# Artessay/RAGraph

Measured on AMD Instinct MI355X. Metric: retrieved-queries/sec (RAGraph_node forward: GCN encode + cosine/top-k retrieval + 3-hop propagate + decode), higher is better.
Workload: dtype f32 (exact results; candidates pre-filtered on bf16 / int8 MFMA with proven bounds)

## Files before the change

ragraph_amd/csrc/filter_prepare.h:

```cpp

constexpr int FILTER_STATS_INTS = 32;
constexpr int FILTER_STATS_MAGIC = 0x52414753;
__device__ __forceinline__ void note_candidates(int* cstat, int64_t b, int n) {
  if (cstat && (b & 63) == 0) {
    atomicAdd(cstat, n);
    atomicAdd(cstat + 3, 1);
  }
}
struct FilterStatsInit {
  int nlev, i8[3], keys[3];
};

constexpr int FILTER_FIX_MAX_Q = 1024;
constexpr int FILTER_FIX_SLICES = 16;

template <int D, int R = 1>
__global__ void __launch_bounds__(256) filter_prep_kernel(const float* __restrict__ Q, int64_t B, float* __restrict__ Qn,
                                                          float* __restrict__ eq, int* __restrict__ count,
                                                          unsigned char* __restrict__ flag, int* __restrict__ overflow,
                                                          int* __restrict__ gmax, int ngroups,
                                                          uint16_t* __restrict__ Qb, int cstride,
                                                          float* __restrict__ eq8, float* __restrict__ qscale,
                                                          signed char* __restrict__ Qb8, int* __restrict__ fix_done,
                                                          int* __restrict__ stats, FilterStatsInit si,
                                                          float* __restrict__ theta_init, float prior) {
  const int lane = threadIdx.x & 63;
  constexpr int NCH = D / 4;
  const int64_t q_first = ((int64_t)blockIdx.x * 4 + (threadIdx.x >> 6)) * R;
  float4 vpre[R];
#pragma unroll
  for (int rr = 0; rr < R; ++rr) {
    vpre[rr] = make_float4(0.f, 0.f, 0.f, 0.f);
    if (lane < NCH && q_first + rr < B) vpre[rr] = reinterpret_cast<const float4*>(Q + (q_first + rr) * D)[lane];
  }
#pragma unroll
  for (int rr = 0; rr < R; ++rr) {
  const int64_t q = q_first + rr;
  if (q == 0 && lane == 0) *overflow = 0;
  if (q == 0 && lane < FILTER_STATS_INTS && stats) {
    int v = 0;
    if (lane == 0) v = FILTER_STATS_MAGIC;
    else if (lane == 1) v = si.nlev;
    else if (lane >= 8 && lane < 11) v = si.i8[lane - 8];
    else if (lane >= 11 && lane < 14) v = si.keys[lane - 11];
    else if (lane == 14) v = B > INT_MAX ? INT_MAX : (int)B;
    else if (lane == 16) v = theta_init ? 1 : 0;
    else if (lane == 18) v = INT_MAX;
    else if (lane == 19) v = INT_MIN;
    stats[lane] = v;
  }
  if (theta_init && q < B && lane == 0) theta_init[q] = prior;
  if (q < FILTER_FIX_MAX_Q && lane == 0) fix_done[q] = 0;
  if (q >= (Qb ? (B + 31) / 32 * 32 : B)) continue;
  float4 v = vpre[rr];
  float p = 0.f;
  p = fmaf(v.x, v.x, p);
  p = fmaf(v.y, v.y, p);
  p = fmaf(v.z, v.z, p);
  p = fmaf(v.w, v.w, p);
  p = wave_sum_fixed_tree(p);
  const float d = fmaxf(sqrtf(p), 1e-12f);
  v.x = v.x / d; v.y = v.y / d; v.z = v.z / d; v.w = v.w / d;
  if (lane < NCH && q < B) reinterpret_cast<float4*>(Qn + q * D)[lane] = v;
  if (Qb && lane < NCH) {
    const int e0 = 4 * lane, t = e0 >> 5, gg = (e0 >> 3) & 3;
    typedef __bf16 bf16x4 __attribute__((ext_vector_type(4)));
    bf16x4 o;
    o[0] = (__bf16)v.x; o[1] = (__bf16)v.y; o[2] = (__bf16)v.z; o[3] = (__bf16)v.w;
    char* base = reinterpret_cast<char*>(Qb) + ((q >> 4) * (D / 32) + t) * 1024 + (gg * 16 + (int)(q & 15)) * 16 + (e0 & 7) * 2;
    *reinterpret_cast<bf16x4*>(base) = o;
  }
  float e2 = 0.f;
  {
    const float x[4] = {v.x, v.y, v.z, v.w};
#pragma unroll
    for (int e = 0; e < 4; ++e) {
      const float dd = x[e] - (float)(__bf16)x[e];
      e2 = fmaf(dd, dd, e2);
    }
  }
  e2 = wave_sum_any_order(e2);
  float e8 = 0.f, sq = 0.f;
  unsigned am = max(max(__float_as_uint(fabsf(v.x)), __float_as_uint(fabsf(v.y))), max(__float_as_uint(fabsf(v.z)), __float_as_uint(fabsf(v.w))));
  am = wave_max_u32(am);
  if (eq8) {
    sq = __uint_as_float(am) / 127.f;
    unsigned w8 = 0u;
    if (sq > 0.f) {
      const float x[4] = {v.x, v.y, v.z, v.w};
#pragma unroll
      for (int e = 0; e < 4; ++e) {
        const int qi = quantize_i8(x[e], 1.f / sq);
        w8 |= ((unsigned)qi & 0xFFu) << (8 * e);
        const float dd = fmaf(sq, (float)qi, -x[e]);
        e8 = fmaf(dd, dd, e8);
      }
    }
    if (Qb8 && lane < NCH) {
      const int c = lane >> 2;
      char* base = reinterpret_cast<char*>(Qb8) + ((q >> 4) * (D / 64) + (c >> 2)) * 1024 + ((c & 3) * 16 + (int)(q & 15)) * 16 + (lane & 3) * 4;
      *reinterpret_cast<unsigned*>(base) = w8;
    }
    e8 = wave_sum_any_order(e8);
  }
  if (q >= B) continue;
  if (lane == 0) {
    eq[q] = sqrtf(e2) * 1.0000002f;
    flag[q] = am == 0u ? 2 : 0;
    if (am == 0u && stats) atomicAdd(stats + 15, 1);
    if (eq8) {
      eq8[q] = sqrtf(e8) * 1.000001f;
      qscale[q] = sq;
    }
  }
  if (lane < cstride) count[q * cstride + lane] = 0;
  if (gmax)
    for (int gi = lane; gi < ngroups; gi += 64) gmax[q * ngroups + gi] = f2ord(RG_NEG_INF);
  }
}

__global__ void __launch_bounds__(256) filter_theta_kernel(FilterThr t, int64_t B, int init, float* __restrict__ theta) {
  const int64_t q = (int64_t)blockIdx.x * 256 + threadIdx.x;
// ... 78 lines not shown
```

ragraph_amd/csrc/filter_ring.h:

```cpp

#ifdef RG_RING_STAMPS
__device__ unsigned long long g_ring_t[2][2][8];
__device__ unsigned long long g_ring_span[2][2];
__device__ unsigned long long g_ring_max[2][8];
#define RG_RSTAMP(i_)                                                                                     \
  if (threadIdx.x == 0 && first_seg) {                                                                    \
    const unsigned long long now_ = wall_clock64();                                                       \
    if (blockIdx.x == 0 || blockIdx.x == gridDim.x - 1) g_ring_t[BOUND][blockIdx.x != 0][i_] = now_;      \
    if ((i_) == 0) atomicMin(&g_ring_span[BOUND][0], now_);                                               \
    else atomicMax(&g_ring_max[BOUND][i_], now_ - rs_prev);                                               \
    rs_prev = now_;                                                                                       \
  }
static void ring_stamps_report(bool BOUND, bool I8) {
  (void)hipDeviceSynchronize();
  unsigned long long t[2][2][8];
  (void)hipMemcpyFromSymbol(t, HIP_SYMBOL(g_ring_t), sizeof(t));
  for (int b = 0; b < 2; ++b)
    fprintf(stderr, "[ring stamps, %s%s launch, %s workgroup, 10 ns ticks] operands %lld thresholds %lld ring primed %lld stages %lld "
            "flush %lld (entered %lld after workgroup 0)\n", BOUND ? "bound" : "filter", I8 ? " int8" : "", b ? "last" : "first",
            (long long)(t[BOUND][b][1] - t[BOUND][b][0]), (long long)(t[BOUND][b][2] - t[BOUND][b][1]),
            (long long)(t[BOUND][b][3] - t[BOUND][b][2]), (long long)(t[BOUND][b][4] - t[BOUND][b][3]),
            (long long)(t[BOUND][b][5] - t[BOUND][b][4]), (long long)(t[BOUND][b][0] - t[BOUND][0][0]));
  unsigned long long span[2][2], mx[2][8];
  (void)hipMemcpyFromSymbol(span, HIP_SYMBOL(g_ring_span), sizeof(span));
  (void)hipMemcpyFromSymbol(mx, HIP_SYMBOL(g_ring_max), sizeof(mx));
  fprintf(stderr, "[ring stamps, all workgroups] first entry to last exit %lld; longest first-segment phases: operands %lld thresholds %lld "
          "ring primed %lld stages %lld flush %lld\n", (long long)(span[BOUND][1] - span[BOUND][0]), (long long)mx[BOUND][1],
          (long long)mx[BOUND][2], (long long)mx[BOUND][3], (long long)mx[BOUND][4], (long long)mx[BOUND][5]);
  unsigned long long init_span[2][2] = {{~0ull, 0ull}, {~0ull, 0ull}}, zero[2][8] = {};
  (void)hipMemcpyToSymbol(HIP_SYMBOL(g_ring_span), init_span, sizeof(init_span));
  (void)hipMemcpyToSymbol(HIP_SYMBOL(g_ring_max), zero, sizeof(zero));
}
#else
#define RG_RSTAMP(i_)
static void ring_stamps_report(bool, bool) {}
#endif
#ifdef RG_TOPK_TIMING
__device__ unsigned long long g_filter_timing[8];
#define RG_FT(var_) const unsigned long long var_ = __builtin_amdgcn_s_memtime()
static void ring_timing_report(int prof_slot, int D) {
  (void)hipDeviceSynchronize();
  unsigned long long t[8];
  (void)hipMemcpyFromSymbol(t, HIP_SYMBOL(g_filter_timing), sizeof(t));
  const double n = (double)t[5];
  if (n > 0)
    fprintf(stderr, "[filter timing] slot %d D=%d wave-stages=%.0f ticks/stage: wait_full %.1f compute %.1f signal+vmcnt "
            "%.1f wait_free %.1f dma_issue %.1f total %.1f; flushes in the loop: %.0f, %.1f ticks each = %.1f per stage\n",
            prof_slot, D, n, t[0] / n, t[1] / n, t[2] / n, t[3] / n, t[4] / n, (t[0] + t[1] + t[2] + t[3] + t[4]) / n, (double)t[7],
            t[7] ? (double)t[6] / (double)t[7] : 0.0, t[6] / n);
  unsigned long long zero[8] = {0, 0, 0, 0, 0, 0, 0, 0};
  (void)hipMemcpyToSymbol(HIP_SYMBOL(g_filter_timing), zero, sizeof(zero));
}
#else
#define RG_FT(var_)
static void ring_timing_report(int, int) {}
#endif

#ifndef RG_RING_FOLD
#define RG_RING_FOLD 1
#endif
template <int D, int QW, bool BOUND = false, bool I8 = false, bool SCORED = false, bool PIPE = false>
__global__ void __launch_bounds__(512, 2) topk_filter_kernel(FilterParams p) {
  using C = FilterCfg<I8 ? D / 2 : D>;
  static_assert(!PIPE || (I8 && !BOUND && C::KSTEPS >= QW / 16 + 2), "PIPE: int8 filter levels, one step per query group + 2");
  static_assert(!(I8 && BOUND), "the bound pass runs on the bf16 copy");
  static_assert(I8 || !SCORED, "scored lists carry the int8 levels' integer sums");
  static_assert(QW == 32 || QW == 64 || QW == 96 || QW == 128, "two, four, six or eight query groups of 16 per wave");
  constexpr int QT = C::WAVES * QW;
  constexpr int NG = QW / 16;
  constexpr bool FOLD = RG_RING_FOLD && I8 && !PIPE && !BOUND && D == 64;
  if (filter_gate_closed(p.gate)) return;
  extern __shared__ float4 fsmem4[];
  char* smem = reinterpret_cast<char*>(fsmem4);
  unsigned* full = reinterpret_cast<unsigned*>(smem + C::SLOTS * C::STAGE_BYTES);
  unsigned* freec = full + C::SLOTS;
  const unsigned lds_base = (unsigned)(size_t)(lds_void_f*)smem;

  const int tid = threadIdx.x;
  const int lane = tid & 63;
  const int wave = __builtin_amdgcn_readfirstlane(tid >> 6);
  const int j = lane & 15, g = lane >> 4;

  unsigned voff[C::DMAS];
#pragma unroll
  for (int i = 0; i < C::DMAS; ++i) voff[i] = (unsigned)(i * 1024 + lane * 16);
  auto dma_stage = [&](int64_t stage_abs, int slot) {
    const uint64_t goff = (uint64_t)stage_abs * C::STAGE_BYTES + (uint64_t)(C::DMAS * wave * 1024);
    const char* gbase = reinterpret_cast<const char*>(p.Kb) +
                        (((uint64_t)(unsigned)__builtin_amdgcn_readfirstlane((int)(goff >> 32)) << 32) |
                         (uint64_t)(unsigned)__builtin_amdgcn_readfirstlane((int)(unsigned)goff));
#pragma unroll
    for (int i = 0; i < C::DMAS; ++i) {
      const unsigned dst = lds_base + (unsigned)(slot * C::STAGE_BYTES + (C::DMAS * wave + i) * 1024);
      unsigned keep;
      asm volatile(
          "s_mov_b32 %0, m0\n\ts_mov_b32 m0, %2\n\ts_nop 0\n\tglobal_load_lds_dwordx4 %1, %3\n\ts_mov_b32 m0, %0"
          : "=&s"(keep)
          : "v"(voff[i]), "s"(dst), "s"(gbase)
          : "memory");
    }
  };
  const unsigned apos = lds_base + (unsigned)lane * 16u;

  const int x = p.xcd_map ? (int)(blockIdx.x & 7) : 0;
  const int64_t nq = p.xcd_map ? ((p.qtiles - x + 7) >> 3) : p.qtiles;
  const int64_t nq0 = p.xcd_map ? ((p.qtiles + 7) >> 3) : p.qtiles;
  SegmentWalker walker(nq, p.nstages_total, p.wgs_per_group, p.lb_min, 0, p.depth[nq != nq0],
                       p.xcd_map ? (int)(blockIdx.x >> 3) : (int)blockIdx.x);
  Segment seg;
  [[maybe_unused]] bool first_seg = true;
#ifdef RG_RING_STAMPS
  unsigned long long rs_prev = 0;
#endif
  RG_RSTAMP(0);
  while (walker.next(seg)) {
    const int64_t qtile = p.xcd_map ? x + 8 * seg.tile : seg.tile;
    const int64_t q_lo = qtile * QT + wave * QW + j;
    const int64_t st0 = seg.st0;
    const int nstages = (int)(seg.st1 - seg.st0);

    bf16x8 bq[I8 ? 1 : NG][I8 ? 1 : C::KS32];
    i32x4 bqi[I8 ? NG : 1][I8 ? C::KS32 : 1];
    constexpr int TB = C::KS32 < 4 ? C::KS32 : 4;
    if constexpr (I8) {
      if (p.Qb) {
        const int64_t qg0 = (qtile * QT + wave * QW) >> 4;
        const int64_t ngroups16 = ((p.B + 31) / 32 * 32) >> 4;
#pragma unroll
        for (int gq = 0; gq < NG; ++gq) {
          const bool have = qg0 + gq < ngroups16;
          const i32x4* src = reinterpret_cast<const i32x4*>(p.Qb) + ((qg0 + gq) * C::KS32) * 64 + lane;
#pragma unroll
          for (int t = 0; t < C::KS32; ++t) {
            i32x4 z = {0, 0, 0, 0};
            bqi[gq][t] = have ? src[t * 64] : z;
          }
        }
      } else
#pragma unroll
      for (int gq = 0; gq < NG; ++gq) {
        const int64_t qq = q_lo + 16 * gq;
        const int64_t qr = qq < p.B ? qq : p.B - 1;
        const float sq = p.thr.qscale[qr];
        const float inv_sq = sq > 0.f ? 1.f / sq : 0.f;
        const float* r0 = p.Qn + qr * D + 16 * g;
#pragma unroll
        for (int t = 0; t < C::KS32; ++t) {
          float4 u[4];
#pragma unroll
          for (int c = 0; c < 4; ++c) u[c] = *reinterpret_cast<const float4*>(r0 + 64 * t + 4 * c);
#pragma unroll
          for (int c = 0; c < 4; ++c) {
            unsigned w = 0u;
            if (sq > 0.f)
              w = ((unsigned)quantize_i8(u[c].x, inv_sq) & 0xFFu) | (((unsigned)quantize_i8(u[c].y, inv_sq) & 0xFFu) << 8) |
                  (((unsigned)quantize_i8(u[c].z, inv_sq) & 0xFFu) << 16) | (((unsigned)quantize_i8(u[c].w, inv_sq) & 0xFFu) << 24);
            bqi[gq][t][c] = (int)w;
          }
          asm volatile("" : "+v"(bqi[gq][t]));
        }
        asm volatile("" ::: "memory");
      }
    } else if (p.Qb) {
      const int64_t qg0 = (qtile * QT + wave * QW) >> 4;
      const int64_t ngroups16 = ((p.B + 31) / 32 * 32) >> 4;
#pragma unroll
      for (int gq = 0; gq < NG; ++gq) {
        const bool have = qg0 + gq < ngroups16;
        const bf16x8* src = reinterpret_cast<const bf16x8*>(p.Qb) + ((qg0 + gq) * C::KS32) * 64 + lane;
#pragma unroll
        for (int t = 0; t < C::KS32; ++t) {
          bf16x8 z;
#pragma unroll
          for (int e = 0; e < 8; ++e) z[e] = (__bf16)0.f;
          bq[gq][t] = have ? src[t * 64] : z;
        }
      }
    } else
#pragma unroll
    for (int gq = 0; gq < NG; ++gq) {
      const int64_t qq = q_lo + 16 * gq;
      const float* r0 = p.Qn + (qq < p.B ? qq : p.B - 1) * D + 8 * g;
#pragma unroll
      for (int t0 = 0; t0 < C::KS32; t0 += TB) {
#pragma unroll
        for (int t = t0; t < t0 + TB; ++t) {
          const float4 u0 = *reinterpret_cast<const float4*>(r0 + 32 * t), u1 = *reinterpret_cast<const float4*>(r0 + 32 * t + 4);
          bq[gq][t][0] = (__bf16)u0.x; bq[gq][t][1] = (__bf16)u0.y; bq[gq][t][2] = (__bf16)u0.z; bq[gq][t][3] = (__bf16)u0.w;
          bq[gq][t][4] = (__bf16)u1.x; bq[gq][t][5] = (__bf16)u1.y; bq[gq][t][6] = (__bf16)u1.z; bq[gq][t][7] = (__bf16)u1.w;
        }
#pragma unroll
        for (int t = t0; t < t0 + TB; ++t) asm volatile("" : "+v"(bq[gq][t]));
        asm volatile("" ::: "memory");
      }
    }
    RG_RSTAMP(1);
    float thr[NG];
    int thr8[NG], thr8h[NG];
#pragma unroll
// ... 459 lines not shown
```

ragraph_amd/csrc/segment_plan.h:

```cpp
#pragma once
#include <stdint.h>

#if defined(__HIPCC__)
#define RG_HD __host__ __device__
#else
#define RG_HD
#endif

namespace ragraph {

struct Segment {
  int64_t tile;
  int64_t st0, st1;
  int slot;
  int last;
};

struct SegmentWalker {
  static constexpr int MIN_SHARE = 4;

  int64_t NS;
  int W, c, lb_min, warm, depth;
  int64_t rounds, round;
  int64_t t0, nT, c0, nC, lo, hi, bud;
// ... 97 lines not shown
        s.st1 = lo + take;
        s.slot = slot0;
        s.last = (lo + take == hi);
        c0 += nT;
        nC -= nT;
        lo += take;
        ++slot0;
        if (carry + take + warm > worst) worst = carry + take + warm;
        if (lo >= hi) nT = 0;
        if (mine) {
          phase = 3;
          return true;
        }
      }
    }
    if (phase == 2) {
      const int64_t len = hi - lo;
      if (aligned) {
        phase = 3;
        const int64_t ci = c - c0;
        if (ci < 0) return false;
        const int64_t jt = ci / m, piece = ci % m;
        const int64_t a = piece * per;
        if (jt >= nT || a >= len) return false;
        s.tile = t0 + jt;
        s.st0 = lo + a;
        s.st1 = a + per < len ? lo + a + per : hi;
        s.slot = slot0 + (int)piece;
        s.last = (s.st1 == hi);
        return true;
      }
      if (c < c0 || lin >= lin_end) {
        phase = 3;
        return false;
      }
      const int64_t jt = lin / len;
      const int64_t a = lin - jt * len;
      const int64_t b = (a + (lin_end - lin) < len) ? a + (lin_end - lin) : len;
      s.tile = t0 + jt;
      s.st0 = lo + a;
      s.st1 = lo + b;
      s.slot = slot0 + (int)((c - c0) - (jt * len) / Lb);
      s.last = (lo + b == hi);
      lin += b - a;
      return true;
    }
    return false;
  }

  struct Choice {
    int depth;
    int64_t slots;
    int64_t load;
  };

  static inline Choice choose_depth(int64_t nq, int64_t NS, int W, int lb_min, int warm) {
    Choice best = {0, 1, 0};
    int64_t min_load = -1;
    int64_t loads[80], slots[80];
    int nd = 0;
    for (int d = 0; d < 80; ++d) {
      SegmentWalker w(nq, NS, W, lb_min, warm, d, -1);
      Segment s;
      while (w.next(s)) {
      }
      loads[d] = w.worst;
      slots[d] = w.used;
      nd = d + 1;
      if (min_load < 0 || w.worst < min_load) min_load = w.worst;
      if (w.steps < d) break;
    }
    const int64_t whole = (nq / W) * (NS + warm) + min_load;
    for (int d = nd - 1; d >= 0; --d)
      if (loads[d] <= min_load + whole / 256) {
        best.depth = d;
        best.slots = slots[d];
        best.load = loads[d];
        break;
      }
    return best;
  }
};

}
```

ragraph_amd/csrc/topk_filter.hip:

```cpp
#include "filter_common.h"
#include "rescore_common.h"
#include <new>
#include "segment_plan.h"
#include <cmath>
#include <type_traits>

namespace ragraph {

typedef __attribute__((address_space(3))) void lds_void_f;
typedef int i32x4 __attribute__((ext_vector_type(4)));

template <int D_>
struct FilterCfg {
  static constexpr int D = D_;
  static constexpr int WAVES = 8, THREADS = 512;
  static constexpr int ROW_BYTES = D * 2;
  static constexpr int CR = D / 8;
  static constexpr int KSTEPS = D / 16;
  static constexpr int KS32 = D / 32;
  static constexpr int STAGE_BYTES = FILTER_STAGE_BYTES;
  static constexpr int STAGE_KEYS = STAGE_BYTES / ROW_BYTES;
  static constexpr int SUBS = STAGE_KEYS / 32;
  static constexpr int NSTEP = SUBS * KSTEPS;
  static constexpr int SLOTS = 4;
// ... 259 lines not shown
  f.part_s = B <= 64 ? reinterpret_cast<float*>(take((size_t)B * 8 * k * sizeof(float))) : nullptr;
  f.part_i = B <= 64 ? reinterpret_cast<int*>(take((size_t)B * 8 * k * sizeof(int))) : nullptr;
  f.eq8 = reinterpret_cast<float*>(take((size_t)B * sizeof(float)));
  f.qscale = reinterpret_cast<float*>(take((size_t)B * sizeof(float)));
  f.Qb8 = B <= FILTER_QB_MAX_B ? reinterpret_cast<signed char*>(take((size_t)((B + 31) / 32 * 32) * D)) : nullptr;
  if (out) *out = f;
  return off;
}

static int filter_shape_code(int64_t B, int64_t N, int D, int k) {
  if (!filter_dim_ok(D)) return RAGRAPH_EUNSUPPORTED;
  return B >= 1 && N >= 1 && k >= 1 && k <= 32 && k <= N ? RAGRAPH_OK : RAGRAPH_EINVAL;
}
#define RG_REQUIRE_FILTER_SHAPE(who, B, N, D, k)                                                                      \
  do {                                                                                                                \
    const int code__ = filter_shape_code(B, N, D, k);                                                                 \
    RG_REQUIRE(code__ != RAGRAPH_EUNSUPPORTED, RAGRAPH_EUNSUPPORTED, who ": D=%d not in {64,128,256}", D);           \
    RG_REQUIRE(code__ == RAGRAPH_OK, RAGRAPH_EINVAL, who ": bad B/N/k");                                              \
  } while (0)

static FilterShape filter_query_shape(int64_t B, int64_t N, int D, int k, int n_shards, bool exchange) {
  return {B, N, N, D, k, n_shards, exchange, __builtin_nanf(""), -1, false, filter_env(), filter_device_cus(), __builtin_nanf("")};
}
static void filter_query_follow_tight(FilterShape& in) {
  if (t_prior == t_prior && t_tight == t_tight && t_tight > t_prior) {
    in.prior = t_prior;
    in.tight = t_tight;
  }
}

static size_t filter_workspace_bytes(FilterShape in, const FilterSchedule& sc) {
  const FilterCall planned = filter_call_plan(in, sc);
  in.exact_level0 = true;
  const FilterCall exact0 = filter_call_plan(in, sc);
  return (planned.level0_bytes > exact0.level0_bytes ? planned.level0_bytes : exact0.level0_bytes) +
         filter_ws_carve(nullptr, in, planned, nullptr) + FILTER_STATS_BYTES;
}
static size_t filter_workspace_bytes(int64_t B, int64_t N, int D, int k, int n_shards) {
  if (B < 1 || N < 1 || k < 1 || n_shards < 1 || !filter_dim_ok(D)) return 0;
  const FilterShape in = filter_query_shape(B, N, D, k, n_shards, n_shards > 1);
  return filter_workspace_bytes(in, filter_schedule(in));
}

extern "C" size_t ragraph_topk_cosine_filtered_workspace_bytes(int64_t B, int64_t N, int D, int k) {
  return filter_workspace_bytes(B, N, D, k, 1);
}
extern "C" size_t ragraph_topk_cosine_filtered_sharded_workspace_bytes(int64_t B, int64_t plan_N, int D, int k, int n_shards) {
  if (!filter_dim_ok(D)) return 0;
  const size_t a = filter_workspace_bytes(B, plan_N, D, k, n_shards), b = filter_workspace_bytes(B, plan_N, D, k, 1);
  const size_t c = ragraph_topk_cosine_workspace_bytes(B, plan_N, D, k);
  const size_t ab = a > b ? a : b;
  return ab > c ? ab : c;
}

extern "C" int ragraph_topk_cosine_filtered_i8_levels(int64_t B, int64_t N, int D, int k) {
  if (filter_shape_code(B, N, D, k) != RAGRAPH_OK) return 0;
  FilterShape in = filter_query_shape(B, N, D, k, 1, false);
  in.i8_cap = t_max_i8_levels;
  filter_query_follow_tight(in);
  return filter_call_plan(in, filter_schedule(in)).i8_levels;
}

extern "C" int ragraph_topk_cosine_filtered_plan(int64_t B, int64_t N, int D, int k, int64_t plan[7]) {
  RG_REQUIRE(plan, RAGRAPH_EINVAL, "topk_cosine_filtered_plan: null pointer");
  RG_REQUIRE_FILTER_SHAPE("topk_cosine_filtered_plan", B, N, D, k);
  FilterShape in = filter_query_shape(B, N, D, k, 1, false);
  filter_query_follow_tight(in);
  const FilterCall c = filter_call_plan(in, filter_schedule(in));
  plan[0] = c.n0;
  plan[1] = c.level0 == FILTER_L0_BOUND ? 2 : (c.level0 == FILTER_L0_SLAB ? 1 : 0);
  plan[2] = c.nlev;
  for (int l = 0; l < FILTER_MAX_LEVELS; ++l) plan[3 + l] = l < c.nlev ? c.level[l].key1 : 0;
  plan[6] = c.bound_keys;
  return c.nlev;
}

extern "C" int ragraph_topk_cosine_filtered_sharded_speculates(int64_t B, int64_t plan_N, int D, int k, int n_shards) {
  if (filter_shape_code(B, plan_N, D, k) != RAGRAPH_OK || n_shards < 1) return 0;
  FilterShape in = filter_query_shape(B, plan_N, D, k, n_shards, true);
  in.prior = 0.f;
  return filter_call_plan(in, filter_schedule(in)).spec ? 1 : 0;
}

template <int D, int QW, bool BOUND, bool I8 = false, bool SCORED = false, bool PIPE = false>
static int launch_ring(FilterParams p, int64_t B, int CUS, int prof_slot, hipStream_t st) {
  using C = FilterCfg<I8 ? D / 2 : D>;
  p.qtiles = cdiv(B, (int64_t)C::WAVES * QW);
  p.xcd_map = p.qtiles >= 64 ? 1 : 0;
  p.wgs_per_group = CUS / (p.xcd_map ? 8 : 1);
  {
    const int64_t per_wg = p.qtiles * p.nstages_total / CUS;
    p.lb_min = per_wg >= 16 ? 8 : (per_wg >= 8 ? 4 : (per_wg >= 3 ? 2 : 1));
  }
  const int64_t nq0 = p.xcd_map ? (p.qtiles + 7) / 8 : p.qtiles;
  for (int v = 0; v < 2; ++v) {
    const int64_t nq = nq0 - v;
    p.depth[v] = 0;
    if (nq < 1 || (v == 1 && (!p.xcd_map || p.qtiles % 8 == 0))) continue;
    p.depth[v] = SegmentWalker::choose_depth(nq, p.nstages_total, p.wgs_per_group, p.lb_min, 0).depth;
    if (p.qtiles * p.nstages_total / CUS < 16) p.depth[v] = 0;
  }
  static DeviceOnce lds_once;
  if (hipError_t e = raise_dynamic_lds(lds_once, &topk_filter_kernel<D, QW, BOUND, I8, SCORED, PIPE>, (int)C::LDS_BYTES); e != hipSuccess) {
    set_error("topk_cosine_filtered: cannot raise dynamic LDS limit: %s", hipGetErrorString(e));
    return RAGRAPH_EDEVICE;
  }
  if (t_prof && prof_slot >= 0) (void)hipEventRecord(t_prof->ev[2 * prof_slot], st);
  hipLaunchKernelGGL((topk_filter_kernel<D, QW, BOUND, I8, SCORED, PIPE>), dim3((unsigned)CUS), dim3(C::THREADS), C::LDS_BYTES, st, p);
  if (t_prof && prof_slot >= 0) (void)hipEventRecord(t_prof->ev[2 * prof_slot + 1], st);
  RG_CHECK_LAUNCH("topk_cosine_filtered(filter)");
  ring_stamps_report(BOUND, I8);
  if (prof_slot >= 0) ring_timing_report(prof_slot, D);
  return RAGRAPH_OK;
}

struct PassVariant {
  bool direct;
  int qw;
  bool bound, i8, scored, pipe;
};
static PassVariant filter_pass_variant(int D, int64_t B, int64_t key0, int64_t key1, bool bound, bool int8, bool scored, int cus,
                                       const FilterEnv& env) {
  PassVariant v{};
  v.qw = 64;
  v.bound = bound;
  v.i8 = int8;
  v.scored = int8 && scored;
  if (B <= 256) {
    v.direct = true;
    return v;
  }
  const int64_t nstages = cdiv(key1 - key0, FILTER_STAGE_BYTES / ((int8 ? 1 : 2) * D));
  auto long_stream = [&](int64_t tile) { return cdiv(B, tile) * nstages >= 32 * (int64_t)cus; };
  if (!int8) {
    if (!bound && D == 64 && B >= 1024 && long_stream(1024)) v.qw = 128;
    return v;
  }
  const int64_t pad64 = cdiv(B, (int64_t)512) * 512 - B;
  auto fits = [&](int64_t tile) {
    return long_stream(tile) && (cdiv(B, tile) * tile - B - pad64) * 50 <= B;
  };
  const int qw = env.i8_qw ? env.i8_qw : (D == 64 && fits(1024) ? 128 : (fits(768) ? 96 : 64));
  const bool long128 = qw == 128 && long_stream(1024), long96 = qw == 96 && long_stream(768);
  if (D == 256 && ((env.pipe == 1 && !long128 && !long96) || env.pipe == 2)) v.pipe = true;
  else v.qw = long128 ? 128 : (long96 ? 96 : 64);
  return v;
}

template <int D>
static int launch_ring_variant(const PassVariant& v, const FilterParams& p, int64_t B, int cus, int prof_slot, hipStream_t st) {
  RG_REQUIRE(!v.direct && (v.qw == 64 || (v.i8 ? !v.pipe && (v.qw == 96 || v.qw == 128) : D == 64 && !v.bound && v.qw == 128)) &&
             (!v.pipe || (D == 256 && v.i8)), RAGRAPH_EINVAL, "topk_cosine_filtered: no ring kernel for D=%d qw=%d bound=%d int8=%d pipe=%d",
             D, v.qw, (int)v.bound, (int)v.i8, (int)v.pipe);
  if (v.bound) return launch_ring<D, 64, true>(p, B, cus, prof_slot, st);
  if (!v.i8) {
    if constexpr (D == 64)
      if (v.qw == 128) return launch_ring<D, 128, false>(p, B, cus, prof_slot, st);
    return launch_ring<D, 64, false>(p, B, cus, prof_slot, st);
  }
  if constexpr (D == 256)
    if (v.pipe)
      return v.scored ? launch_ring<D, 64, false, true, true, true>(p, B, cus, prof_slot, st)
                      : launch_ring<D, 64, false, true, false, true>(p, B, cus, prof_slot, st);
#define RG_RING_I8(QW_) \
  return v.scored ? launch_ring<D, QW_, false, true, true>(p, B, cus, prof_slot, st) : launch_ring<D, QW_, false, true>(p, B, cus, prof_slot, st)
  if (v.qw == 128) RG_RING_I8(128);
  if (v.qw == 96) RG_RING_I8(96);
  RG_RING_I8(64);
#undef RG_RING_I8
}

template <int D>
static int run_pass(const FilterWs& f, const uint16_t* Kb, const signed char* Kb8, int64_t B, int64_t key0, int64_t key1,
                    const FilterThr& thr, int cap, int bound_groups, bool int8, bool scored, const FilterEnv& env, int cus,
                    int prof_slot, hipStream_t st, FilterGate gate = FilterGate{nullptr, 0, 0}) {
  const PassVariant v = filter_pass_variant(D, B, key0, key1, bound_groups > 0, int8, scored, cus, env);
  const uint16_t* keys = v.i8 ? reinterpret_cast<const uint16_t*>(Kb8) : Kb;
  const uint16_t* Qimg = v.i8 ? reinterpret_cast<const uint16_t*>(f.Qb8) : f.Qb;
  if (v.direct) {
    DirectArgs a{};
    a.Qb = Qimg;
    a.Kb = keys;
    a.i8 = v.i8;
    a.scored = v.scored;
// ... 178 lines not shown
  r.f.theta = r.theta;
  r.f.overflow_list = f.overflow_list;
  r.f.fix_done = f.fix_done;
  return r;
}

template <int D>
static int run_tight_repair(const FilteredArgs& a, const FilterCall& c, const FilterShape& in, const FilterWs& f, FilterThr thr,
                            const signed char* K8, int* stats, hipStream_t st) {
  const int64_t B = a.B, N = a.N;
  const int k = a.k;
  const FilterLevel& lv = c.level[c.nlev - 1];
  const size_t slot = c.scored_slots ? sizeof(int2) : sizeof(int);
  RG_REQUIRE((size_t)(reinterpret_cast<char*>(f.theta) - reinterpret_cast<char*>(f.cand)) >= filter_repair_bytes(D, k, slot),
             RAGRAPH_EWORKSPACE, "topk_cosine_filtered: the repair's buffers do not fit the idle lists");
  const FilterRepairWs r = filter_repair_carve(f, D, k, lv.int8, slot);
  hipLaunchKernelGGL(filter_tight_verdict_kernel, dim3((unsigned)cdiv(B, 256)), dim3(256), 0, st, a.out_scores, a.out_idx, B, k,
                     in.tight, in.prior, f.flag, f.theta, r.list, stats);
  RG_CHECK_LAUNCH("topk_cosine_filtered(soft verdict)");
  hipLaunchKernelGGL(filter_repair_gather_kernel<D>, dim3(FILTER_REPAIR_Q), dim3(64), 0, st, a.Q, f.theta, r.list, r.Q, r.theta, stats);
  RG_CHECK_LAUNCH("topk_cosine_filtered(repair gather)");
  hipLaunchKernelGGL((filter_prep_kernel<D, 1>), dim3(FILTER_REPAIR_Q / 4), dim3(256), 0, st, r.Q, (int64_t)FILTER_REPAIR_Q, r.f.Qn,
                     r.f.eq, r.f.count, r.f.flag, r.dummy, (int*)nullptr, k, r.f.Qb, filter_count_stride(FILTER_REPAIR_Q),
                     lv.int8 ? r.f.eq8 : nullptr, r.f.qscale, r.f.Qb8, r.f.fix_done, (int*)nullptr, FilterStatsInit{},
                     (float*)nullptr, 0.f);
  RG_CHECK_LAUNCH("topk_cosine_filtered(repair prepare)");
  FilterThr thr2 = thr;
  thr2.theta = r.theta;
  thr2.prev_scores = nullptr;
  thr2.gmax = nullptr;
  thr2.eq = r.f.eq;
  thr2.eq8 = r.f.eq8;
  thr2.qscale = r.f.qscale;
  thr2.flag = r.f.flag;
  int rc = run_pass<D>(r.f, a.Kb, K8, FILTER_REPAIR_Q, 0, N, thr2, FILTER_LIST_CAP, 0, lv.int8, c.repair_scored, in.env, in.cus, -1, st,
                       FilterGate{stats + 22, 1, FILTER_REPAIR_Q});
  if (rc != RAGRAPH_OK) return rc;
  rc = run_rescore<D>(r.f, a.Kn, N, FILTER_REPAIR_Q, FILTER_LIST_CAP, k, 0, 0, 0, r.out_s, r.out_i, r.dummy,
                      rescore_kind(FILTER_REPAIR_Q, k, c.repair_scored, false), thr2, nullptr, st);
  if (rc != RAGRAPH_OK) return rc;
  hipLaunchKernelGGL(filter_repair_scatter_kernel, dim3(FILTER_REPAIR_Q), dim3(64), 0, st, r.list, r.out_s, r.out_i, r.f.flag, k,
                     a.out_scores, a.out_idx, f.flag, stats);
  RG_CHECK_LAUNCH("topk_cosine_filtered(repair scatter)");
  thr.theta = f.theta;
  thr.gmax = nullptr;
  thr.prev_scores = a.out_scores;
  rc = run_pass<D>(f, a.Kb, K8, B, 0, N, thr, c.cap, 0, lv.int8, lv.scored, in.env, in.cus, -1, st,
                   FilterGate{stats + 22, FILTER_REPAIR_Q + 1, INT_MAX});
  if (rc != RAGRAPH_OK) return rc;
  return run_rescore<D>(f, a.Kn, N, B, c.cap, k, a.idx_base, 1, 1, a.out_scores, a.out_idx, a.overflow,
                        rescore_kind(B, k, lv.scored, false), thr, nullptr, st);
}

template <int D>
static int run_filtered(const FilteredArgs& a, const FilterCall& c, const FilterShape& in) {
  hipStream_t st = as_stream(a.stream);
  const int64_t B = a.B, N = a.N;
  const int k = a.k;
  float* const out_scores = a.out_scores;
  int64_t* const out_idx = a.out_idx;
  const bool sharded = a.exchange != nullptr, bound = c.level0 == FILTER_L0_BOUND;
  static const int ablate = [] {
    const char* e = getenv("RAGRAPH_FILTER_ABLATE");
    return e ? atoi(e) : 0;
  }();
  if (t_prof) t_prof->have = t_prof->bound = 0;

  char* w = static_cast<char*>(a.ws);
  FilterWs f;
  const size_t used = c.level0_bytes + filter_ws_carve(w + c.level0_bytes, in, c, &f) + FILTER_STATS_BYTES;
  RG_REQUIRE(used <= a.ws_bytes, RAGRAPH_EWORKSPACE, "topk_cosine_filtered: the schedule of this call needs %zu bytes of workspace, "
             "%zu given", used, a.ws_bytes);
  int* stats = reinterpret_cast<int*>(w + ragraph_topk_cosine_filtered_stats_offset(a.ws_bytes));
  const unsigned* max_kerr2 = reinterpret_cast<const unsigned*>(a.Kb + filter_round_up(N) * D);
  const FilterI8View v8 = filter_i8_view(a.Kb, N, D);

  FilterStatsInit stats_init{};
  stats_init.nlev = c.nlev;
  for (int l = 0; l < c.nlev; ++l) {
    stats_init.i8[l] = c.level[l].int8;
    const int64_t lk = c.level[l].key1 - c.level[l].key0;
    stats_init.keys[l] = lk > INT_MAX ? INT_MAX : (int)lk;
  }
#define RG_PREP(R_)                                                                                                                     \
  hipLaunchKernelGGL((filter_prep_kernel<D, R_>), dim3((unsigned)cdiv(B <= FILTER_QB_MAX_B ? (B + 31) / 32 * 32 : B, 4 * (R_))), dim3(256), 0, st, a.Q, B, \
                     f.Qn, f.eq, f.count, f.flag, a.overflow, bound ? f.gmax : nullptr, c.parts, c.bf16_image ? f.Qb : nullptr,         \
                     filter_count_stride(B), c.i8_levels > 0 ? f.eq8 : nullptr, f.qscale, B <= FILTER_QB_MAX_B ? f.Qb8 : nullptr, f.fix_done, \
                     stats, stats_init, c.spec ? (sharded ? a.theta : f.theta) : nullptr, c.tight ? in.tight : in.prior)
  if (B >= 8192) RG_PREP(4);
  else RG_PREP(1);
#undef RG_PREP
  RG_CHECK_LAUNCH("topk_cosine_filtered(prepare)");

  FilterThr thr{};
  thr.eq = f.eq;
  thr.max_kerr2 = max_kerr2;
  thr.eq8 = f.eq8;
  thr.qscale = f.qscale;
  thr.tail8 = v8.tail8;
  thr.cls8 = v8.cls;
  thr.flag = f.flag;
  thr.k = k;
  thr.ngroups = c.parts;
  thr.ablate = ablate;
  int rc = RAGRAPH_OK;
  switch (c.level0) {
    case FILTER_L0_NONE: break;
    case FILTER_L0_BOUND:
      rc = run_pass<D>(f, a.Kb, v8.K8, B, 0, c.bound_keys, thr, c.cap, c.parts, false, false, in.env, in.cus, 3, st);
      if (t_prof) {
        t_prof->bound = 1;
        t_prof->i8[3] = 0;
        t_prof->keys[3] = c.bound_keys;
      }
      break;
    case FILTER_L0_SLAB: {
      float* S = reinterpret_cast<float*>(w);
      for (int64_t b0 = 0; b0 < B && rc == RAGRAPH_OK; b0 += FILTER_SLAB_MAX_B) {
        const int64_t nb = B - b0 < FILTER_SLAB_MAX_B ? B - b0 : FILTER_SLAB_MAX_B;
        rc = ragraph_linear_f32(f.Qn + b0 * D, nb, D, a.Kn, c.n0, nullptr, RAGRAPH_ACT_NONE, 0.f, S, a.stream);
        if (rc == RAGRAPH_OK)
          rc = ragraph_topk_rows_f32(S, nb, c.n0, c.n0, k, out_scores + b0 * k, out_idx + b0 * k, a.stream);
      }
      break;
    }
    case FILTER_L0_TILE:
      rc = ragraph_topk_cosine_bank_f32(a.Q, B, a.Kn, D == 256 ? a.Kp : nullptr, c.n0, D, k, 0, out_scores, out_idx, a.ws,
                                        c.level0_bytes, a.stream);
      break;
  }
  if (rc != RAGRAPH_OK) return rc;
  if (sharded && c.spec) {
    thr.theta = a.theta;
  } else if (sharded) {
    thr.gmax = bound ? f.gmax : nullptr;
    thr.prev_scores = out_scores;
    if (bound) {
      hipLaunchKernelGGL(filter_bound_scores_kernel, dim3((unsigned)cdiv(B, 4)), dim3(256), 0, st, thr, B, out_scores, a.theta);
      RG_CHECK_LAUNCH("topk_cosine_filtered(theta)");
    } else if ((rc = launch_theta(thr, B, 1, a.theta, st)) != RAGRAPH_OK) {
      return rc;
    }
    a.exchange(a.ctx, 0);
    thr.theta = a.theta;
  } else if (bound && c.parts > k) {
    thr.gmax = f.gmax;
    hipLaunchKernelGGL(filter_bound_scores_kernel, dim3((unsigned)cdiv(B, 4)), dim3(256), 0, st, thr, B, (float*)nullptr, f.theta);
    RG_CHECK_LAUNCH("topk_cosine_filtered(theta)");
  }

  for (int l = 0; l < c.nlev; ++l) {
    const FilterLevel& lv = c.level[l];
    thr.gmax = (l == 0 && bound && !sharded && c.parts == k) ? f.gmax : nullptr;
    if (!sharded) thr.theta = (c.spec || (l == 0 && bound && c.parts > k)) ? f.theta : nullptr;
    thr.prev_scores = out_scores;
    rc = run_pass<D>(f, a.Kb, v8.K8, B, lv.key0, lv.key1, thr, c.cap, 0, lv.int8, lv.scored, in.env, in.cus, l, st);
    if (t_prof) {
      t_prof->i8[l] = lv.int8;
      t_prof->keys[l] = lv.key1 - lv.key0;
    }
    if (rc != RAGRAPH_OK) return rc;
    if (t_prof) t_prof->have = l + 1;
    rc = run_rescore<D>(f, a.Kn, N, B, c.cap, k, a.idx_base, l > 0, l == c.level_final, out_scores, out_idx, a.overflow,
                        rescore_kind(B, k, lv.scored, sharded && l > 0), thr, stats + 2 + l, st);
    if (rc != RAGRAPH_OK) return rc;
    if (l + 1 == c.nlev) break;
// ... 88 lines not shown
```

Baseline: 5.413 million.

## Add split ring schedule that balances ragged XCD tiles across all CUs

```diff
diff --git a/ragraph_amd/csrc/filter_prepare.h b/ragraph_amd/csrc/filter_prepare.h
--- a/ragraph_amd/csrc/filter_prepare.h
+++ b/ragraph_amd/csrc/filter_prepare.h
@@ -37,7 +37,7 @@
   for (int rr = 0; rr < R; ++rr) {
   const int64_t q = q_first + rr;
   if (q == 0 && lane == 0) *overflow = 0;
-  if (q == 0 && lane < FILTER_STATS_INTS && stats) {
+  if (q == 0 && lane < FILTER_STATS_INTS && lane != 15 && stats) {
     int v = 0;
     if (lane == 0) v = FILTER_STATS_MAGIC;
     else if (lane == 1) v = si.nlev;
diff --git a/ragraph_amd/csrc/filter_ring.h b/ragraph_amd/csrc/filter_ring.h
--- a/ragraph_amd/csrc/filter_ring.h
+++ b/ragraph_amd/csrc/filter_ring.h
@@ -102,11 +102,7 @@
   };
   const unsigned apos = lds_base + (unsigned)lane * 16u;
 
-  const int x = p.xcd_map ? (int)(blockIdx.x & 7) : 0;
-  const int64_t nq = p.xcd_map ? ((p.qtiles - x + 7) >> 3) : p.qtiles;
-  const int64_t nq0 = p.xcd_map ? ((p.qtiles + 7) >> 3) : p.qtiles;
-  SegmentWalker walker(nq, p.nstages_total, p.wgs_per_group, p.lb_min, 0, p.depth[nq != nq0],
-                       p.xcd_map ? (int)(blockIdx.x >> 3) : (int)blockIdx.x);
+  RingWalker walker(p.qtiles, p.nstages_total, p.wgs_per_group, p.lb_min, p.xcd_map, p.depth[0], p.depth[1], (int)blockIdx.x);
   Segment seg;
   [[maybe_unused]] bool first_seg = true;
 #ifdef RG_RING_STAMPS
@@ -114,7 +110,7 @@
 #endif
   RG_RSTAMP(0);
   while (walker.next(seg)) {
-    const int64_t qtile = p.xcd_map ? x + 8 * seg.tile : seg.tile;
+    const int64_t qtile = walker.qtile(seg);
     const int64_t q_lo = qtile * QT + wave * QW + j;
     const int64_t st0 = seg.st0;
     const int nstages = (int)(seg.st1 - seg.st0);
diff --git a/ragraph_amd/csrc/segment_plan.h b/ragraph_amd/csrc/segment_plan.h
--- a/ragraph_amd/csrc/segment_plan.h
+++ b/ragraph_amd/csrc/segment_plan.h
@@ -203,4 +203,77 @@
   }
 };
 
+enum { RING_ONE = 0, RING_XCD = 1, RING_SPLIT = 2 };
+
+struct RingWalker {
+  SegmentWalker w;
+  int64_t tile0;
+  int tstride;
+  int64_t left, left0;
+  int cus, bid, depth_left;
+
+  RG_HD RingWalker(int64_t qtiles, int64_t NS, int W, int lb_min, int mode, int depth0, int depth1, int bid_)
+      : w(group_tiles(qtiles, mode, bid_), NS, W, lb_min, 0,
+          (mode == RING_XCD && group_tiles(qtiles, mode, bid_) != ((qtiles + 7) >> 3)) ? depth1 : depth0,
+          mode == RING_ONE ? bid_ : bid_ >> 3),
+        tile0(mode == RING_ONE ? 0 : (bid_ & 7)),
+        tstride(mode == RING_ONE ? 1 : 8),
+        left(mode == RING_SPLIT ? (qtiles & 7) : 0),
+        left0((qtiles >> 3) << 3),
+        cus(mode == RING_ONE ? W : 8 * W),
+        bid(bid_),
+        depth_left(depth1) {}
+
+  static RG_HD int64_t group_tiles(int64_t qtiles, int mode, int b) {
+    return mode == RING_ONE ? qtiles : (mode == RING_XCD ? (qtiles - (b & 7) + 7) >> 3 : qtiles >> 3);
+  }
+
+  RG_HD bool next(Segment& s) {
+    while (!w.next(s)) {
+      if (!left) return false;
+      w = SegmentWalker(left, w.NS, cus, w.lb_min, 0, depth_left, bid);
+      tile0 = left0;
+      tstride = 1;
+      left = 0;
+    }
+    return true;
+  }
+  RG_HD int64_t qtile(const Segment& s) const { return tile0 + tstride * s.tile; }
+};
+
+struct RingPlan {
+  int mode, depth[2];
+  int64_t load;
+};
+
+static inline int64_t ring_plan_load(int64_t qtiles, int64_t NS, int CUS, int lb_min, const RingPlan& pl) {
+  int64_t worst = 0;
+  for (int b = 0; b < CUS; ++b) {
+    RingWalker rw(qtiles, NS, pl.mode == RING_ONE ? CUS : CUS / 8, lb_min, pl.mode, pl.depth[0], pl.depth[1], b);
+    Segment s;
+    int64_t load = 0;
+    while (rw.next(s)) load += s.st1 - s.st0;
+    if (load > worst) worst = load;
+  }
+  return worst;
 }
+
+static inline RingPlan ring_plan_choose(int64_t qtiles, int64_t NS, int CUS, int lb_min) {
+  const bool xcd = qtiles >= 64;
+  const int W = CUS / (xcd ? 8 : 1);
+  const bool shallow = qtiles * NS / CUS < 16;
+  auto depth_of = [&](int64_t nq, int Wg) {
+    return (nq < 1 || shallow) ? 0 : SegmentWalker::choose_depth(nq, NS, Wg, lb_min, 0).depth;
+  };
+  RingPlan pl{xcd ? RING_XCD : RING_ONE, {0, 0}, 0};
+  const int64_t nq0 = xcd ? (qtiles + 7) / 8 : qtiles;
+  pl.depth[0] = depth_of(nq0, W);
+  if (!xcd || qtiles % 8 == 0) return pl;
+  pl.depth[1] = depth_of(nq0 - 1, W);
+  RingPlan sp{RING_SPLIT, {pl.depth[1], depth_of(qtiles % 8, CUS)}, 0};
+  pl.load = ring_plan_load(qtiles, NS, CUS, lb_min, pl);
+  sp.load = ring_plan_load(qtiles, NS, CUS, lb_min, sp);
+  return sp.load < pl.load ? sp : pl;
+}
+
+}
diff --git a/ragraph_amd/csrc/topk_filter.hip b/ragraph_amd/csrc/topk_filter.hip
--- a/ragraph_amd/csrc/topk_filter.hip
+++ b/ragraph_amd/csrc/topk_filter.hip
@@ -365,24 +365,36 @@
   return filter_call_plan(in, filter_schedule(in)).spec ? 1 : 0;
 }
 
+static RingPlan ring_plan_cached(int64_t qtiles, int64_t NS, int CUS, int lb_min) {
+  struct Entry {
+    int64_t qtiles, NS;
+    int CUS, lb_min;
+    RingPlan pl;
+  };
+  constexpr int SLOTS = 16;
+  thread_local Entry cache[SLOTS];
+  thread_local int used = 0, victim = 0;
+  for (int i = 0; i < used; ++i)
+    if (cache[i].qtiles == qtiles && cache[i].NS == NS && cache[i].CUS == CUS && cache[i].lb_min == lb_min) return cache[i].pl;
+  const RingPlan pl = ring_plan_choose(qtiles, NS, CUS, lb_min);
+  const int at = used < SLOTS ? used++ : (victim = (victim + 1) % SLOTS);
+  cache[at] = Entry{qtiles, NS, CUS, lb_min, pl};
+  return pl;
+}
+
 template <int D, int QW, bool BOUND, bool I8 = false, bool SCORED = false, bool PIPE = false>
 static int launch_ring(FilterParams p, int64_t B, int CUS, int prof_slot, hipStream_t st) {
   using C = FilterCfg<I8 ? D / 2 : D>;
   p.qtiles = cdiv(B, (int64_t)C::WAVES * QW);
-  p.xcd_map = p.qtiles >= 64 ? 1 : 0;
-  p.wgs_per_group = CUS / (p.xcd_map ? 8 : 1);
   {
     const int64_t per_wg = p.qtiles * p.nstages_total / CUS;
     p.lb_min = per_wg >= 16 ? 8 : (per_wg >= 8 ? 4 : (per_wg >= 3 ? 2 : 1));
   }
-  const int64_t nq0 = p.xcd_map ? (p.qtiles + 7) / 8 : p.qtiles;
-  for (int v = 0; v < 2; ++v) {
-    const int64_t nq = nq0 - v;
-    p.depth[v] = 0;
-    if (nq < 1 || (v == 1 && (!p.xcd_map || p.qtiles % 8 == 0))) continue;
-    p.depth[v] = SegmentWalker::choose_depth(nq, p.nstages_total, p.wgs_per_group, p.lb_min, 0).depth;
-    if (p.qtiles * p.nstages_total / CUS < 16) p.depth[v] = 0;
-  }
+  const RingPlan pl = ring_plan_cached(p.qtiles, p.nstages_total, CUS, p.lb_min);
+  p.xcd_map = pl.mode;
+  p.wgs_per_group = CUS / (pl.mode == RING_ONE ? 1 : 8);
+  p.depth[0] = pl.depth[0];
+  p.depth[1] = pl.depth[1];
   static DeviceOnce lds_once;
   if (hipError_t e = raise_dynamic_lds(lds_once, &topk_filter_kernel<D, QW, BOUND, I8, SCORED, PIPE>, (int)C::LDS_BYTES); e != hipSuccess) {
     set_error("topk_cosine_filtered: cannot raise dynamic LDS limit: %s", hipGetErrorString(e));
@@ -727,6 +739,10 @@
     const int64_t lk = c.level[l].key1 - c.level[l].key0;
     stats_init.keys[l] = lk > INT_MAX ? INT_MAX : (int)lk;
   }
+  if (hipMemsetAsync(stats + 15, 0, sizeof(int), st) != hipSuccess) {
+    set_error("topk_cosine_filtered: memset failed");
+    return RAGRAPH_EDEVICE;
+  }
 #define RG_PREP(R_)                                                                                                                     \
   hipLaunchKernelGGL((filter_prep_kernel<D, R_>), dim3((unsigned)cdiv(B <= FILTER_QB_MAX_B ? (B + 31) / 32 * 32 : B, 4 * (R_))), dim3(256), 0, st, a.Q, B, \
                      f.Qn, f.eq, f.count, f.flag, a.overflow, bound ? f.gmax : nullptr, c.parts, c.bf16_image ? f.Qb : nullptr,         \
```

After: 5.561 million, median of 6. +2.7%, better.
